# paipaoso/pytorch-operator-1

Hardware: AMD Instinct MI355X
Metric: samples/sec MNIST DDP (higher is better)
Workload: dtype fp32; 1 GPU; model=mnist-cnn (reference examples/mnist/mnist.py Net, 431,080 params), global_batch=64, per_rank_batch=64, optimizer=SGD lr=0.01 momentum=0.5, parallelism=dp1, impl=fused, sampler=none (every rank its own batch stream, reference-equivalent), backend=none

## Files before the change

### pytorch_operator_1_amd/csrc/kernels/mnist_kernels.hip

```cpp
#include <stdlib.h>

#include "mfma_f32.h"
#include "sgd_f32.h"
#include "xgmi_ar.h"

#ifndef PTO_STAMP
#define PTO_STAMP(k) ((void)0)
#define PTO_STAMP_SCOPE()
#endif

namespace {

constexpr int C1 = 20, C2 = 50, P1 = 12, F1OUT = 500, F1IN = 800, NCLS = 10;
constexpr int A1P = C1 * P1 * P1;

PTO_DEV void relu_pool4(const float v[4], float& out, uint8_t& code) {
  float m = v[0];
  int a = 0;
#pragma unroll
  for (int r = 1; r < 4; ++r)
    if (v[r] > m) { m = v[r]; a = r; }
  if (m > 0.f) { out = m; code = (uint8_t)a; }
  else { out = 0.f; code = 4; }
}
// ... 1232 lines not shown
          const bool ok = (unsigned)sy < 8u && (unsigned)sx < 8u;
          tv[kh * 5 + kw] = ts[(icl * 25 + kh * 5 + kw) * TLD + (ok ? sy * 8 + sx : 0)];
          tv[kh * 5 + kw] = ok ? tv[kh * 5 + kw] : 0.f;
        }
      float sacc = 0.f;
#pragma unroll
      for (int t = 0; t < 25; ++t) sacc += tv[t];
      if (da1p) da1p[b * A1P + (icg * 2 + icl) * 144 + pix] = sacc;
      dsum[o] = sacc;
    }
    {
      const int o = 256 + (tid >> 3), part = tid & 7, pix = o - 144;
      const int y = pix / 12, xx = pix - y * 12;
      float tv[4];
#pragma unroll
      for (int i = 0; i < 4; ++i) {
        const int tt = part + 8 * i;
        const int kh = tt / 5, kw = tt - kh * 5, sy = y - kh, sx = xx - kw;
        const bool ok = tt < 25 && (unsigned)sy < 8u && (unsigned)sx < 8u;
        tv[i] = ts[(25 + (tt < 25 ? tt : 0)) * TLD + (ok ? sy * 8 + sx : 0)];
        tv[i] = ok ? tv[i] : 0.f;
      }
      float sacc = tv[0];
      sacc += tv[1];
      sacc += tv[2];
      sacc += tv[3];
      sacc += lane_mirror8(sacc);
      sacc += lane_xor2(sacc);
      sacc += lane_xor1(sacc);
      if (part == 0) {
        if (da1p) da1p[b * A1P + (icg * 2 + 1) * 144 + pix] = sacc;
        dsum[o] = sacc;
      }
    }
  }
  if (!fuse1) return;
  __syncthreads();
  PTO_STAMP(4);
  float* part = ws;
  {
    const int icl = wv >> 1, p0 = (wv & 1) * 72;
    float acc[26];
#pragma unroll
    for (int k = 0; k < 26; ++k) acc[k] = 0.f;
#pragma unroll
    for (int it = 0; it < 2; ++it) {
      const int pl = lane + 64 * it;
      if (pl < 72) {
        const int pix = p0 + pl;
        const int cd = c1s[icl * 144 + pix];
        const float v = cd < 4 ? dsum[icl * 144 + pix] : 0.f;
        const int oh = 2 * (pix / 12) + ((cd >> 1) & 1), ow = 2 * (pix % 12) + (cd & 1);
        const float* xp = xs + oh * 28 + ow;
#pragma unroll
        for (int kh = 0; kh < 5; ++kh)
#pragma unroll
          for (int kw = 0; kw < 5; ++kw) acc[kh * 5 + kw] = fmaf(v, xp[kh * 28 + kw], acc[kh * 5 + kw]);
        acc[25] += v;
      }
    }
    wave_halving26(acc, lane, part + wv * 26);
  }
  __syncthreads();
  PTO_STAMP(5);
  if (tid < 52) {
    const int icl = tid / 26, k = tid - icl * 26, oc1 = icg * 2 + icl;
    const float v = part[(2 * icl) * 26 + k] + part[(2 * icl + 1) * 26 + k];
    if (det) {
      if (k < 25) gw1[oc1 * 25 + k] = v;
      else gb1[oc1] = v;
    } else {
      if (k < 25) atomicAdd(gw1 + oc1 * 25 + k, v);
      else atomicAdd(gb1 + oc1, v);
    }
  }
}

PTO_DEV float c2_bias_sum(int oc, const float* __restrict__ g2, const uint8_t* __restrict__ code2, int B) {
  const int lane = threadIdx.x & 63;
  float s = 0.f;
  for (int i0 = 0; i0 < B * 16; i0 += 64 * 8) {
    float gv[8];
    int cd[8];
#pragma unroll
    for (int q = 0; q < 8; ++q) {
      const int i = i0 + q * 64 + lane;
      const int idx = (i >> 4) * F1IN + oc * 16 + (i & 15);
      const bool ok = i < B * 16;
      gv[q] = ok ? g2[idx] : 0.f;
      cd[q] = ok ? (int)code2[idx] : 4;
    }
#pragma unroll
    for (int q = 0; q < 8; ++q) s += cd[q] < 4 ? gv[q] : 0.f;
  }
  return wave_sum(s);
}

__global__ __launch_bounds__(256) void k_conv2_bwd(const float* __restrict__ g2, const uint8_t* __restrict__ code2,
                                                   const float* __restrict__ a1p, const float* __restrict__ w2,
                                                   float* __restrict__ gw2, float* __restrict__ gb2,
                                                   float* __restrict__ da1p, int B, int nA, int nB, int nC,
                                                   const float* __restrict__ x, const long long* __restrict__ bidx,
                                                   const uint8_t* __restrict__ code1, float* __restrict__ gw1,
                                                   float* __restrict__ gb1) {
  extern __shared__ __attribute__((aligned(16))) float smem[];
  int bid = blockIdx.x;
  const int wv = threadIdx.x >> 6, lane = threadIdx.x & 63;
  if (bid < nA) {
    c2_wgrad_block<B2_CHUNK>(bid, smem, g2, code2, a1p, gw2, B);
    return;
  }
  bid -= nA;
  if (bid < nB) {
    c2_dgrad_block(bid, smem, g2, code2, w2, da1p, B, x, bidx, code1, gw1, gb1, false);
    return;
  }
  bid -= nB;
  if (bid < nC) {
    const int oc = bid * 4 + wv;
    if (oc >= C2) return;
    const float s = c2_bias_sum(oc, g2, code2, B);
    if (lane == 0) gb2[oc] = s;
  }
}

PTO_DEV void dw1_sgd_tile(int tile, const float* __restrict__ dh1, const float* __restrict__ a2p,
                          float* __restrict__ pw, float* __restrict__ mw, int B, const SgdArgs& a) {
  constexpr int MT = (F1OUT + 15) / 16, NT = (F1IN + 15) / 16;
  if (tile >= MT * NT) return;
  const int mt = tile % MT, nt = tile / MT, lane = threadIdx.x & 63;
  const int n = nt * 16 + (lane & 15);
  float pv[4], mv[4];
#pragma unroll
  for (int rr = 0; rr < 4; ++rr) {
    const int r = mt * 16 + (lane >> 4) * 4 + rr;
    const bool ok = r < F1OUT && n < F1IN;
    pv[rr] = ok ? pw[r * F1IN + n] : 0.f;
    mv[rr] = ok ? mw[r * F1IN + n] : 0.f;
  }
  const float lr = *a.lr;
  const f32x4 acc =
      wave_tile_16x16<LAY_KROW, LAY_KROW, 4>(dh1, F1OUT, a2p, F1IN, F1OUT, F1IN, B, mt * 16, nt * 16, 0, B);
#pragma unroll
  for (int rr = 0; rr < 4; ++rr) {
    const int r = mt * 16 + (lane >> 4) * 4 + rr;
    if (r < F1OUT && n < F1IN) {
      sgd_elem(pv[rr], acc[rr], mv[rr], lr, a.mom, a.wd, a.gscale, a.nesterov);
      pw[r * F1IN + n] = pv[rr];
      mw[r * F1IN + n] = mv[rr];
    }
  }
}

PTO_DEV void dw1_tile_pair(int pair, const float* __restrict__ dh1, const float* __restrict__ a2p,
                           float* __restrict__ pw, float* __restrict__ mw, float* __restrict__ gout, int B,
                           const SgdArgs& a) {
  constexpr int MT = (F1OUT + 15) / 16, NT = (F1IN + 15) / 16;
  static_assert(NT % 2 == 0 && F1IN % 16 == 0, "dW1 column tiles pair up with no column tail");
  if (pair >= MT * NT / 2) return;
  const int mt = pair % MT, nt0 = 2 * (pair / MT), lane = threadIdx.x & 63;
  const int r = lane & 15, g = lane >> 4;
  float pv[2][4], mv[2][4];
  if (!gout) {
#pragma unroll
    for (int t = 0; t < 2; ++t)
#pragma unroll
      for (int rr = 0; rr < 4; ++rr) {
        const int row = mt * 16 + g * 4 + rr, n = (nt0 + t) * 16 + r;
        const bool ok = row < F1OUT;
        pv[t][rr] = ok ? pw[row * F1IN + n] : 0.f;
        mv[t][rr] = ok ? mw[row * F1IN + n] : 0.f;
      }
  }
  f32x4 acc[2][2] = {{zero4(), zero4()}, {zero4(), zero4()}};
  constexpr int NG = 4;
  for (int k = 0; k < B; k += 16 * NG) {
    float av[NG][4], bv[2][NG][4];
#pragma unroll
    for (int q = 0; q < NG; ++q) {
      load4<LAY_KROW>(dh1, F1OUT, mt * 16 + r, F1OUT, k + 16 * q + 4 * g, B, av[q]);
#pragma unroll
      for (int t = 0; t < 2; ++t) load4<LAY_KROW>(a2p, F1IN, (nt0 + t) * 16 + r, F1IN, k + 16 * q + 4 * g, B, bv[t][q]);
    }
#pragma unroll
    for (int q = 0; q < NG; ++q)
#pragma unroll
      for (int j = 0; j < 4; ++j)
#pragma unroll
        for (int t = 0; t < 2; ++t) acc[t][j & 1] = mfma16x16x4(av[q][j], bv[t][q][j], acc[t][j & 1]);
  }
  const float lr = gout ? 0.f : *a.lr;
#pragma unroll
  for (int t = 0; t < 2; ++t) {
    const f32x4 s = acc[t][0] + acc[t][1];
#pragma unroll
    for (int rr = 0; rr < 4; ++rr) {
      const int row = mt * 16 + g * 4 + rr, n = (nt0 + t) * 16 + r;
      if (row >= F1OUT) continue;
      if (gout) {
        gout[row * F1IN + n] = s[rr];
      } else {
        sgd_elem(pv[t][rr], s[rr], mv[t][rr], lr, a.mom, a.wd, a.gscale, a.nesterov);
        pw[row * F1IN + n] = pv[t][rr];
        mw[row * F1IN + n] = mv[t][rr];
      }
    }
  }
}

constexpr int B1_CHUNK = 4;
PTO_DEV void conv1_bwd_block(int vb, const float* __restrict__ g1, const uint8_t* __restrict__ code1,
                             const float* __restrict__ x, float* __restrict__ gw1, float* __restrict__ gb1, int B,
                             const long long* __restrict__ bidx) {
  __shared__ __attribute__((aligned(16))) float xs[B1_CHUNK * 784];
  __shared__ float part[4][26];
  x = batch_ptr(x, bidx, B * 784);
  const int oc = vb % C1, chunk = vb / C1;
  const int b0 = chunk * B1_CHUNK, nb = min(B, b0 + B1_CHUNK) - b0;
  const int nitems = nb * 144;
  constexpr int PER = (B1_CHUNK * 144 + 255) / 256;
  constexpr int XPER = (B1_CHUNK * 196 + 255) / 256;
  float gv[PER];
  int cd[PER];
  float4 xv[XPER];
#pragma unroll
  for (int q = 0; q < XPER; ++q) {
    const int e = threadIdx.x + 256 * q;
    xv[q] = e < nb * 196 ? reinterpret_cast<const float4*>(x + b0 * 784)[e] : float4{0.f, 0.f, 0.f, 0.f};
  }
#pragma unroll
  for (int q = 0; q < PER; ++q) {
    const int it = threadIdx.x + 256 * q;
    const bool ok = it < nitems;
    const int idx = ok ? ((b0 + it / 144) * C1 + oc) * 144 + it % 144 : 0;
    gv[q] = ok ? g1[idx] : 0.f;
    cd[q] = ok ? (int)code1[idx] : 4;
  }
#pragma unroll
  for (int q = 0; q < XPER; ++q) {
    const int e = threadIdx.x + 256 * q;
    if (e < B1_CHUNK * 196) reinterpret_cast<float4*>(xs)[e] = xv[q];
  }
  __syncthreads();
  float acc[26];
#pragma unroll
  for (int k = 0; k < 26; ++k) acc[k] = 0.f;
#pragma unroll
  for (int q = 0; q < PER; ++q) {
    const int it = threadIdx.x + 256 * q;
    if (cd[q] >= 4) continue;
    const int smp = it / 144, pix = it - smp * 144;
    const int oh = 2 * (pix / 12) + (cd[q] >> 1), ow = 2 * (pix % 12) + (cd[q] & 1);
    const float* xp = xs + smp * 784 + oh * 28 + ow;
    const float gq = gv[q];
#pragma unroll
    for (int kh = 0; kh < 5; ++kh)
#pragma unroll
      for (int kw = 0; kw < 5; ++kw) acc[kh * 5 + kw] = fmaf(gq, xp[kh * 28 + kw], acc[kh * 5 + kw]);
    acc[25] += gq;
  }
  const int wv = threadIdx.x >> 6, lane = threadIdx.x & 63;
  wave_halving26(acc, lane, part[wv]);
  __syncthreads();
  if (threadIdx.x < 26) {
    const int q = threadIdx.x;
    const float s = part[0][q] + part[1][q] + part[2][q] + part[3][q];
    if (q < 25) atomicAdd(gw1 + oc * 25 + q, s);
    else atomicAdd(gb1 + oc, s);
  }
}

__global__ __launch_bounds__(256) void k_conv1_bwd(const float* __restrict__ g1, const uint8_t* __restrict__ code1,
                                                   const float* __restrict__ x, float* __restrict__ gw1,
                                                   float* __restrict__ gb1, int B,
                                                   const long long* __restrict__ bidx) {
  conv1_bwd_block(blockIdx.x, g1, code1, x, gw1, gb1, B, bidx);
}

#ifndef PTO_BWD_DTPW
#define PTO_BWD_DTPW 1
#endif
constexpr int BWD_DTPW = PTO_BWD_DTPW;
static int bwd_dpair() {
  static int v = -1;
  if (v < 0) {
    const char* e = getenv("PTO_BWD_DPAIR");
    v = (e && BWD_DTPW == 1) ? (atoi(e) != 0) : 0;
  }
  return v;
}
#ifndef PTO_BWD_ORDER
#define PTO_BWD_ORDER 0
#endif
__host__ __device__ constexpr int bwd_order(int i) {
  constexpr int o[6][5] = {{0, 1, 2, 3, 4}, {3, 2, 4, 0, 1}, {3, 2, 0, 1, 4}, {2, 3, 0, 1, 4},
                           {3, 4, 2, 0, 1}, {0, 1, 3, 2, 4}};
  return o[PTO_BWD_ORDER][i];
}
constexpr int bwd_n_dw1_blocks(bool pair) {
  return pair ? ((((F1OUT + 15) / 16) * ((F1IN + 15) / 16) / 2) + 3) / 4
              : ((((F1OUT + 15) / 16) * ((F1IN + 15) / 16) + 3) / 4 + BWD_DTPW - 1) / BWD_DTPW;
}

struct BwdAllArgs {
  const float* g2;
  const uint8_t* code2;
  const float* a1p;
  const float* w2f;
  const float* x;
  const uint8_t* code1;
  float* gw1;
  float* gb1;
  float* p2w; float* g2w; float* m2w;
  int* ctr;
  float* p2b; float* m2b;
  const float* dh1; const float* a2p; const float* h1; const float* dl;
  float* p1w; float* m1w;
  float* p1b; float* m1b;
  float* pfw; float* mfw;
  float* pfb; float* mfb;
  SgdArgs a;
  long long* bidx;
  long long nbatches;
  int* pending;
  int B, nA, nB, nC, nD, nF;
  int dpair;
  float* wpart;
  float* c1rep;
  int nrep, rep_stride, bias_off;
  int grads_only;
  float* g2b; float* g1w; float* g1b; float* gfw; float* gfb;
  float* hz;
  int nz;
};

struct EpiSgd {
  float* p; float* m; int ld; float lr; const SgdArgs* a;
  PTO_DEV void operator()(int r, int c, float g) const {
    const int i = r * ld + c;
    float pv = p[i], mv = m[i];
    sgd_elem(pv, g, mv, lr, a->mom, a->wd, a->gscale, a->nesterov);
    p[i] = pv;
    m[i] = mv;
  }
};

template <int CH, int NTW>
__global__ __launch_bounds__(256) void k_bwd_all(BwdAllArgs A) {
  extern __shared__ __attribute__((aligned(16))) float smem[];
  __shared__ int s_last;
  int bid = blockIdx.x;
  PTO_STAMP_SCOPE();
  const int wv = threadIdx.x >> 6, lane = threadIdx.x & 63;
  if (bid == 0 && threadIdx.x == 0) {
    if (A.bidx) *A.bidx = (*A.bidx + 1) % A.nbatches;
    if (A.pending) *A.pending = 1;
  }
  if (A.hz) {
    const int i = bid * 256 + (int)threadIdx.x;
    if (i < A.nz) A.hz[i] = 0.f;
  }
  int role = 4;
  {
    const int cnt[5] = {A.nC, A.nF, A.nA, A.nB, A.nD};
#pragma unroll
    for (int i = 0; i < 5; ++i) {
      const int r = bwd_order(i);
      if (bid < cnt[r]) {
        role = r;
        break;
      }
      bid -= cnt[r];
    }
  }
  if (role == 0) {
    const int oc = bid * 4 + wv;
    if (oc >= C2) return;
    const float g = c2_bias_sum(oc, A.g2, A.code2, A.B);
    if (lane == 0 && A.grads_only) A.g2b[oc] = g;
    else if (lane == 0) {
      float pv = A.p2b[oc], mv = A.m2b[oc];
      sgd_elem(pv, g, mv, *A.a.lr, A.a.mom, A.a.wd, A.a.gscale, A.a.nesterov);
      A.p2b[oc] = pv;
      A.m2b[oc] = mv;
    }
    return;
  }
  if (role == 1) {
    const float lr = *A.a.lr;
    constexpr int NWF = (((NCLS + 15) / 16) * ((F1OUT + 15) / 16) + 3) / 4;
    if (A.grads_only) {
      if (bid < NWF) {
        block_gemm_4tiles<LAY_KROW, LAY_KROW>(A.dl, NCLS, A.h1, F1OUT, NCLS, F1OUT, A.B, bid, EpiStore{A.gfw, F1OUT});
        return;
      }
      bid -= NWF;
      if (bid < 8) block_colsum64(A.dh1, F1OUT, A.B, F1OUT, bid * 64, smem, A.g1b);
      else block_colsum64(A.dl, NCLS, A.B, NCLS, 0, smem, A.gfb);
      return;
    }
    if (bid < NWF) {
      block_gemm_4tiles<LAY_KROW, LAY_KROW>(A.dl, NCLS, A.h1, F1OUT, NCLS, F1OUT, A.B, bid,
                                            EpiSgd{A.pfw, A.mfw, F1OUT, lr, &A.a});
      return;
    }
    bid -= NWF;
    if (bid < 8) block_colsum64_epi(A.dh1, F1OUT, A.B, F1OUT, bid * 64, smem, EpiSgd{A.p1b, A.m1b, 0, lr, &A.a});
    else block_colsum64_epi(A.dl, NCLS, A.B, NCLS, 0, smem, EpiSgd{A.pfb, A.mfb, 0, lr, &A.a});
    return;
  }
  if (role == 2) {
    const bool det = A.wpart != nullptr;
    c2_wgrad_block<CH, NTW>(bid, smem, A.g2, A.code2, A.a1p, A.g2w, A.B, A.wpart);
    if (A.grads_only && !det) return;
    asm volatile("s_waitcnt vmcnt(0)" ::: "memory");
    __syncthreads();
    PTO_STAMP(3);
    constexpr int NT = 32 / NTW, TC = 16 * NTW;
    const int nt = bid % NT, nchunk = A.nA / NT;
    if (threadIdx.x == 0) {
      if (det) __builtin_amdgcn_fence(__ATOMIC_RELEASE, "agent");
      const int old = __hip_atomic_fetch_add(A.ctr + nt, 1, __ATOMIC_RELAXED, __HIP_MEMORY_SCOPE_AGENT);
      s_last = old == nchunk - 1;
      if (s_last) {
        __hip_atomic_store(A.ctr + nt, 0, __ATOMIC_RELAXED, __HIP_MEMORY_SCOPE_AGENT);
        if (det) __builtin_amdgcn_fence(__ATOMIC_ACQUIRE, "agent");
      }
    }
    __syncthreads();
    PTO_STAMP(4);
    if (!s_last) return;
    constexpr int NQ = (C2 * TC + 255) / 256;
    int idx[NQ];
    float gv[NQ], pv[NQ], mv[NQ];
    if (det) {
#pragma unroll
      for (int q = 0; q < NQ; ++q) {
        const int e = threadIdx.x + 256 * q, row = e / TC, col = nt * TC + (e % TC);
        idx[q] = (e < C2 * TC && col < 500) ? row * 500 + col : -1;
        float g = 0.f;
        if (idx[q] >= 0)
          for (int c = 0; c < nchunk; ++c) g += A.wpart[c * (C2 * 500) + idx[q]];
        gv[q] = g;
      }
      if (A.grads_only) {
#pragma unroll
        for (int q = 0; q < NQ; ++q)
          if (idx[q] >= 0) A.g2w[idx[q]] = gv[q];
        return;
      }
    }
    const float lr = *A.a.lr;
#pragma unroll
    for (int q = 0; q < NQ; ++q) {
      const int e = threadIdx.x + 256 * q, row = e / TC, col = nt * TC + (e % TC);
      idx[q] = (e < C2 * TC && col < 500) ? row * 500 + col : -1;
      if (idx[q] >= 0) {
        if (!det) gv[q] = atomicExch(A.g2w + idx[q], 0.f);
        pv[q] = A.p2w[idx[q]];
        mv[q] = A.m2w[idx[q]];
      }
    }
#pragma unroll
    for (int q = 0; q < NQ; ++q)
      if (idx[q] >= 0) {
        sgd_elem(pv[q], gv[q], mv[q], lr, A.a.mom, A.a.wd, A.a.gscale, A.a.nesterov);
        A.p2w[idx[q]] = pv[q];
        A.m2w[idx[q]] = mv[q];
      }
    return;
  }
  if (role == 3) {
    const int r = (bid / B2_ICG) % A.nrep;
    float* gw1 = r == 0 ? A.gw1 : A.c1rep + (r - 1) * A.rep_stride;
    float* gb1 = r == 0 ? A.gb1 : A.c1rep + (r - 1) * A.rep_stride + A.bias_off;
    c2_dgrad_block(bid, smem, A.g2, A.code2, A.w2f, nullptr, A.B, A.x, nullptr, A.code1, gw1, gb1,
                   A.wpart != nullptr);
    return;
  }
  if (role == 4) {
    if (A.dpair) {
      dw1_tile_pair(bid * 4 + wv, A.dh1, A.a2p, A.p1w, A.m1w, A.grads_only ? A.g1w : nullptr, A.B, A.a);
      return;
    }
#pragma unroll
    for (int j = 0; j < BWD_DTPW; ++j) {
      const int vb = bid * BWD_DTPW + j;
      if (A.grads_only)
        block_gemm_4tiles<LAY_KROW, LAY_KROW, EpiStore, 4>(A.dh1, F1OUT, A.a2p, F1IN, F1OUT, F1IN, A.B, vb,
                                                          EpiStore{A.g1w, F1IN});
      else
        dw1_sgd_tile(vb * 4 + wv, A.dh1, A.a2p, A.p1w, A.m1w, A.B, A.a);
    }
    return;
  }
}

__global__ __launch_bounds__(256) void k_conv1_commit(Conv1Commit cm, int* __restrict__ pending) {
  const int pend = *cm.pending;
  const float lr = *cm.a.lr;
  if (!pend) return;
  for (int i = 4 * threadIdx.x; i < cm.n; i += 1024) commit4(cm, i, lr);
  __syncthreads();
  if (threadIdx.x == 0) *pending = 0;
}

__global__ __launch_bounds__(256) void k_ddp_sgd(float* __restrict__ p, float* __restrict__ g, float* __restrict__ m,
                                                 int n, int c1, int zero_from, float* __restrict__ rep, int nrep,
                                                 SgdArgs a, long long* __restrict__ bidx, long long nbatches) {
  if (bidx && blockIdx.x == 0 && threadIdx.x == 0) *bidx = (*bidx + 1) % nbatches;
  const int i = (blockIdx.x * 256 + threadIdx.x) * 4;
  if (i >= n) return;
  const float lr = *a.lr;
  if (i >= c1) {
    const Conv1Commit cm{p + c1, g + c1, m + c1, n - c1, nullptr, a, rep, nrep, n - c1};
    commit4(cm, i - c1, lr);
  } else {
    sgd_flat4(p, g, m, i, lr, a, i >= zero_from);
  }
}

__global__ __launch_bounds__(256) void k_conv1_bwd_data(const float* __restrict__ g1,
                                                        const uint8_t* __restrict__ code1,
                                                        const float* __restrict__ w, float* __restrict__ dx, int B) {
  const int idx = blockIdx.x * 256 + threadIdx.x;
  if (idx >= B * 784) return;
  const int b = idx / 784, pix = idx - b * 784, y = pix / 28, xx = pix - (pix / 28) * 28;
  float s = 0.f;
  for (int oc = 0; oc < C1; ++oc)
    for (int kh = 0; kh < 5; ++kh) {
      const int oh = y - kh;
      if (oh < 0 || oh >= 24) continue;
      for (int kw = 0; kw < 5; ++kw) {
        const int ow = xx - kw;
        if (ow < 0 || ow >= 24) continue;
        const int pi = ((b * C1 + oc) * 12 + (oh >> 1)) * 12 + (ow >> 1);
        if (code1[pi] == ((oh & 1) * 2 + (ow & 1))) s = fmaf(g1[pi], w[oc * 25 + kh * 5 + kw], s);
      }
    }
  dx[idx] = s;
}

__global__ __launch_bounds__(256) void k_eval_head(const float* __restrict__ logp, const int64_t* __restrict__ labels,
                                                   float* __restrict__ stats, int B) {
  const int row = blockIdx.x * 256 + threadIdx.x;
  float loss = 0.f, corr = 0.f;
  if (row < B) {
    const float* z = logp + row * NCLS;
    int am = 0;
    float mv = z[0];
    for (int c = 1; c < NCLS; ++c)
      if (z[c] > mv) { mv = z[c]; am = c; }
    const int y = (int)labels[row];
    loss = -z[y];
    corr = (am == y) ? 1.f : 0.f;
  }
  loss = wave_sum(loss);
  corr = wave_sum(corr);
  if ((threadIdx.x & 63) == 0) {
    atomicAdd(stats, loss);
    atomicAdd(stats + 1, corr);
  }
}

}

#define PTO_API extern "C" __attribute__((visibility("default")))
#define LAUNCH_CHECK() return (int)hipGetLastError()

PTO_API int pto_conv1_fwd(const float* x, const float* w, const float* b, float* out, uint8_t* code, int B,
                          const long long* bidx, hipStream_t s) {
  hipLaunchKernelGGL(k_conv1_fwd, dim3((B * 720 + 255) / 256), dim3(256), 0, s, x, w, b, out, code, B, bidx);
  LAUNCH_CHECK();
}

PTO_API int pto_conv2_fwd(const float* a1p, const float* w, const float* b, float* out, uint8_t* code, int B,
                          hipStream_t s) {
  hipLaunchKernelGGL(k_conv2_fwd, dim3(B * 4), dim3(256), 0, s, a1p, w, b, out, code, B);
  LAUNCH_CHECK();
}

static SgdArgs sgd_args(const float* lr, float mom, float wd, float gscale, int nesterov) {
  SgdArgs a;
  a.lr = lr;
  a.mom = mom;
  a.wd = wd;
  a.gscale = gscale;
  a.nesterov = nesterov;
  a.variant = 0;
  return a;
}

PTO_API int pto_conv12_fwd_lazy_x(const float* x, const float* w1, const float* b1, const float* w2,
                                  const float* b2, float* a1p, uint8_t* code1, float* a2p, uint8_t* code2, int B,
                                  const long long* bidx, const float* g1f, const float* m1f, int bias_off,
                                  const int* pending, const float* lr, float mom, float wd, float gscale, int nesterov,
                                  float* xout, float* w2out, const float* rep, int nrep, int rep_stride,
                                  hipStream_t s) {
  if (nrep < 1 || nrep > C1_MAXREP || (nrep > 1 && !rep) || (pending && (!g1f || !m1f || !lr))) return -1;
  LazyConv1 lz{g1f, m1f, pending, sgd_args(lr, mom, wd, gscale, nesterov), bias_off, xout, w2out, rep, nrep,
               rep_stride};
  hipLaunchKernelGGL(HIP_KERNEL_NAME(k_conv12_fwd2_t<1024, 0>), dim3(B * 4), dim3(1024), 0, s, x, w1, b1, w2, b2, a1p,
                     code1, a2p, code2, B, bidx, lz, ArRole{}, ArRole{});
  LAUNCH_CHECK();
}

extern "C" long long pto_ar_timeout_ticks();

PTO_API int pto_conv12_fwd_ar(const float* x, const float* w1, const float* b1, const float* w2, const float* b2,
                              float* a1p, uint8_t* code1, float* a2p, uint8_t* code2, int B, const long long* bidx,
                              float* xout, const void* peers, int rank, int world, void* epochs, void* err,
                              int protocol, float* p, float* m, const float* lr, float mom, float wd, float gscale,
                              int nesterov, long long fc_off, long long fc_n, int fc_chan, long long fc_zero_from,
                              long long cv_off, long long cv_n, int cv_chan, long long rep_base, int nrep,
                              int rep_stride, long long rep_from, int* ready, hipStream_t s) {
  using namespace pto_ar;
  if (fc_n <= AR_ONESHOT_MAX || fc_n % 4 || fc_off % 4 || fc_n > (1LL << 29) || cv_n > AR_ONESHOT_MAX || cv_n < 4 ||
      cv_n % 4 || cv_off % 4 || world < 1 || world > AR_MAX_RANKS || fc_chan < 0 || fc_chan >= AR_CHANNELS ||
      cv_chan < 0 || cv_chan >= AR_CHANNELS || fc_chan == cv_chan || rank < 0 || rank >= world || !p || !m || !lr ||
      !peers || !ready || protocol < 0 || protocol > 1 || B < 0 || ((((uintptr_t)p) | ((uintptr_t)m)) & 15))
    return -1;
  if (nrep < 1 || nrep > AR_MAX_REP || (nrep > 1 && (rep_stride % 4 || rep_from % 4 || rep_base % 4 ||
                                                      rep_base < cv_off + cv_n || rep_from < cv_off ||
                                                      rep_from + rep_stride > cv_off + cv_n)))
    return -1;
  LazyConv1 lz{nullptr, nullptr, nullptr, sgd_args(lr, mom, wd, gscale, nesterov), 0, xout, nullptr, nullptr, 1, 0};
  ArRole ar{}, cv{};
  for (ArRole* r : {&ar, &cv}) {
    r->peers = reinterpret_cast<const ArPeers*>(peers);
    r->rank = rank;
    r->world = world;
    r->epochs = reinterpret_cast<uint32_t*>(epochs);
    r->err = reinterpret_cast<int*>(err);
    r->timeout = pto_ar_timeout_ticks();
    r->f = ArSgd{};
    r->f.p = p;
    r->f.m = m;
    r->f.a = sgd_args(lr, mom, wd, gscale, nesterov);
    r->f.nbatches = 1;
    r->f.nrep = 1;
    r->ready = ready;
  }
  ar.off = fc_off;
  ar.n4 = fc_n / 4;
  ar.chan = fc_chan;
  ar.nblk = role_blocks(fc_n, world, 1024);
  ar.f.zero_from = fc_zero_from;
  cv.off = cv_off;
// ... 16 lines not shown
  LAUNCH_CHECK();
}

PTO_API int pto_linear_fwd(const float* x, const float* w, const float* b, float* y, int M, int N, int K, int relu,
                           hipStream_t s) {
  const int tiles = ((M + 15) / 16) * ((N + 15) / 16);
  const bool vec = (K % 4) == 0 && ((((uintptr_t)x) | ((uintptr_t)w)) & 15) == 0;
  if (vec)
    hipLaunchKernelGGL(k_linear_fwd_vec16, dim3(tiles), dim3(1024), 0, s, x, w, b, y, M, N, K, relu);
  else
    hipLaunchKernelGGL(k_linear_fwd, dim3(tiles), dim3(256), 0, s, x, w, b, y, M, N, K, relu);
  LAUNCH_CHECK();
}

PTO_API int pto_fc1_fwd_split(const float* x, const float* w, float* h, int M, hipStream_t s) {
  if (M < 1 || !x || !w || !h || ((((uintptr_t)x) | ((uintptr_t)w)) & 15)) return -1;
  static const int nw = [] {
    const char* e = getenv("PTO_FC1_NW");
    const int v = e ? atoi(e) : 16;
    return (v == 4 || v == 8) ? v : 16;
  }();
  const dim3 g(((M + 15) / 16) * 64);
  if (nw == 4)
    hipLaunchKernelGGL(HIP_KERNEL_NAME(k_fc1_fwd_split2<4>), g, dim3(256), 0, s, x, w, h, M);
  else if (nw == 16)
    hipLaunchKernelGGL(HIP_KERNEL_NAME(k_fc1_fwd_split2<16>), g, dim3(1024), 0, s, x, w, h, M);
  else
    hipLaunchKernelGGL(HIP_KERNEL_NAME(k_fc1_fwd_split2<8>), g, dim3(512), 0, s, x, w, h, M);
  LAUNCH_CHECK();
}

PTO_API int pto_linear_bwd(const float* dy, const float* x, const float* w, float* dx, float* dw, float* db, int M,
                           int N, int K, hipStream_t s) {
  if (dx) {
    const int tiles = ((M + 15) / 16) * ((K + 15) / 16);
    hipLaunchKernelGGL(k_linear_bwd_data, dim3(tiles), dim3(256), 0, s, dy, w, dx, M, N, K);
  }
  if (dw) {
    const int tiles = ((N + 15) / 16) * ((K + 15) / 16);
    hipLaunchKernelGGL(k_linear_bwd_weight, dim3((tiles + 3) / 4), dim3(256), 0, s, dy, x, dw, M, N, K);
  }
  if (db) hipLaunchKernelGGL(k_colsum, dim3((N + 63) / 64), dim3(256), 0, s, dy, db, M, N);
  LAUNCH_CHECK();
}

PTO_API int pto_relu_bwd(const float* g, const float* y, float* out, int n, hipStream_t s) {
  hipLaunchKernelGGL(k_relu_bwd, dim3((n + 255) / 256), dim3(256), 0, s, g, y, out, n);
  LAUNCH_CHECK();
}

PTO_API int pto_fc2_ce(const float* h1, const float* w, const float* b, const int64_t* labels, float* logp,
                       float* loss_rows, float* dlogits, float* dh1, int B, float inv_b, const long long* bidx,
                       hipStream_t s) {
  hipLaunchKernelGGL(k_fc2_ce, dim3((B + 3) / 4), dim3(256), 0, s, h1, w, b, labels, logp, loss_rows, dlogits, dh1,
                     B, inv_b, bidx);
  LAUNCH_CHECK();
}

PTO_API int pto_conv1_commit(float* p1, float* g1, float* m1, int n1, int* pending, const float* lr, float mom,
                             float wd, float gscale, int nesterov, float* rep, int nrep, int rep_stride,
                             hipStream_t s) {
  if (n1 % 4 || rep_stride % 4 || ((((uintptr_t)p1) | ((uintptr_t)g1) | ((uintptr_t)m1) | ((uintptr_t)rep)) & 15))
    return -1;
  Conv1Commit cm{p1, g1, m1, n1, pending, sgd_args(lr, mom, wd, gscale, nesterov), rep, nrep, rep_stride};
  hipLaunchKernelGGL(k_conv1_commit, dim3(1), dim3(256), 0, s, cm, pending);
  LAUNCH_CHECK();
}

PTO_API int pto_mnist_ddp_sgd(float* p, float* g, float* m, int n, int c1, int zero_from, float* rep, int nrep,
                              const float* lr, float mom, float wd, float gscale, int nesterov, long long* bidx,
                              long long nbatches, hipStream_t s) {
  if (n % 4 || c1 % 4 || zero_from % 4 || c1 < 0 || c1 >= n || !lr || nrep < 1 || nrep > C1_MAXREP ||
      (nrep > 1 && !rep) || (bidx && nbatches < 1))
    return -1;
  if ((((uintptr_t)p) | ((uintptr_t)g) | ((uintptr_t)m) | ((uintptr_t)rep)) & 15) return -1;
  hipLaunchKernelGGL(k_ddp_sgd, dim3((n / 4 + 255) / 256), dim3(256), 0, s, p, g, m, n, c1, zero_from, rep, nrep,
                     sgd_args(lr, mom, wd, gscale, nesterov), bidx, nbatches);
  LAUNCH_CHECK();
}

PTO_API int pto_conv2_bwd(const float* g2, const uint8_t* code2, const float* a1p, const float* w2, float* gw2,
                          float* gb2, float* da1p, int B, int parts, const float* x, const long long* bidx,
                          const uint8_t* code1, float* gw1, float* gb1, hipStream_t s) {
  if ((parts & 2) && (((uintptr_t)w2) & 7)) return -1;
  const int nA = (parts & 1) ? ((B + B2_CHUNK - 1) / B2_CHUNK) * 32 : 0;
  const int nB = (parts & 2) ? B * B2_ICG : 0;
  const int nC = (parts & 4) ? (C2 + 3) / 4 : 0;
  const size_t ldsA = (parts & 1) ? wgrad_lds_floats<B2_CHUNK, 1>() * sizeof(float) : 0;
  const size_t ldsB = (parts & 2) ? B2_LDS_FLOATS * sizeof(float) : 0;
  const size_t lds = ldsA > ldsB ? ldsA : ldsB;
  if (nA + nB + nC == 0) return 0;
  hipLaunchKernelGGL(k_conv2_bwd, dim3(nA + nB + nC), dim3(256), lds, s, g2, code2, a1p, w2, gw2, gb2, da1p, B, nA,
                     nB, nC, x, bidx, code1, (parts & 2) ? gw1 : nullptr, gb1);
  LAUNCH_CHECK();
}

PTO_API int pto_fc2_ce_dx(const float* h1, const float* w2, const float* b2, const int64_t* labels, const float* w1,
                          float* loss_rows, float* dlogits, float* dh1, float* da2p, int B, float inv_b,
                          const long long* bidx, float* p1, float* g1, float* m1, int n1, const int* pending,
                          const float* lr, float mom, float wd, float gscale, int nesterov, float* rep, int nrep,
                          int rep_stride, int* zero_word, const float* st_x, float* st_xnext, long long st_nb,
                          const float* b1, float* h1out, hipStream_t s) {
  if (b1 && (!h1out || ((((uintptr_t)b1) | ((uintptr_t)h1out)) & 15))) return -1;
  if (n1 % 4 || rep_stride % 4 || ((((uintptr_t)p1) | ((uintptr_t)g1) | ((uintptr_t)m1) | ((uintptr_t)rep)) & 15))
    return -1;
  if ((((uintptr_t)h1) | ((uintptr_t)w2)) & 15) return -1;
  if (nrep < 1 || nrep > C1_MAXREP || (nrep > 1 && !rep)) return -1;
  if (st_xnext && (!st_x || !bidx || st_nb < 1 || ((((uintptr_t)st_x) | ((uintptr_t)st_xnext)) & 15))) return -1;
  Conv1Commit cm{p1, g1, m1, n1, pending, sgd_args(lr, mom, wd, gscale, nesterov), rep, nrep, rep_stride, zero_word};
  const BatchStage st{st_x, st_xnext, st_nb, B * 784 / 4};
  const int nblk = ((B + 15) / 16) * ((F1IN + 15) / 16);
  hipLaunchKernelGGL(k_fc2_ce_dx_mf, dim3(nblk + 1 + (st_xnext ? STAGE_BLOCKS : 0)), dim3(FDX_WAVES * 64), 0, s, h1,
                     w2, b2, labels, w1, loss_rows, dlogits, dh1, da2p, B, inv_b, bidx, cm, st, b1, h1out);
  LAUNCH_CHECK();
}

PTO_API int pto_conv1_bwd(const float* g1, const uint8_t* code1, const float* x, float* gw1, float* gb1, int B,
                          const long long* bidx, hipStream_t s) {
  const int nblk = C1 * ((B + B1_CHUNK - 1) / B1_CHUNK);
  hipLaunchKernelGGL(k_conv1_bwd, dim3(nblk), dim3(256), 0, s, g1, code1, x, gw1, gb1, B, bidx);
  LAUNCH_CHECK();
}

PTO_API int pto_conv1_bwd_data(const float* g1, const uint8_t* code1, const float* w, float* dx, int B,
                               hipStream_t s) {
  hipLaunchKernelGGL(k_conv1_bwd_data, dim3((B * 784 + 255) / 256), dim3(256), 0, s, g1, code1, w, dx, B);
  LAUNCH_CHECK();
}

PTO_API int pto_eval_head(const float* logp, const int64_t* labels, float* stats, int B, hipStream_t s) {
  hipLaunchKernelGGL(k_eval_head, dim3((B + 255) / 256), dim3(256), 0, s, logp, labels, stats, B);
  LAUNCH_CHECK();
}

#ifndef PTO_BWD_WCHUNK
#define PTO_BWD_WCHUNK 5
#endif
constexpr int BWD_WCHUNK = PTO_BWD_WCHUNK;
constexpr int BWD_WNTW = 1;

PTO_API int pto_bwd_all(const float* g2, const uint8_t* code2, const float* a1p, const float* w2f, const float* x,
                        const uint8_t* code1, const float* dh1, const float* a2p, const float* h1, const float* dl,
                        float* p, float* g, float* m, long long off_fc2w, long long off_fc2b, long long off_fc1w,
                        long long off_fc1b, long long off_c2w, long long off_c2b, long long off_c1w,
                        long long off_c1b, int* ctr, long long* bidx, long long nbatches, int* pending, int B,
                        const float* lr, float mom, float wd, float gscale, int nesterov, float* c1rep, int nrep,
                        int rep_stride, int grads_only, float* wpart, float* hz, int nz, hipStream_t s) {
  if (!ctr) return -1;
  if (((uintptr_t)(grads_only ? p + off_c2w : w2f)) & 7) return -1;
  if (!grads_only && (!bidx || !pending || !w2f)) return -1;
  if (bidx && nbatches < 1) return -1;
  if (B < 1 || nrep < 1 || nrep > C1_MAXREP || (nrep > 1 && !c1rep)) return -1;
  if (wpart && nrep != B) return -1;
  BwdAllArgs A;
  A.g2 = g2; A.code2 = code2; A.a1p = a1p; A.w2f = w2f; A.x = x; A.code1 = code1;
  A.gw1 = g + off_c1w; A.gb1 = g + off_c1b;
  A.p2w = p + off_c2w; A.g2w = g + off_c2w; A.m2w = m + off_c2w; A.ctr = ctr;
  A.p2b = p + off_c2b; A.m2b = m + off_c2b;
  A.dh1 = dh1; A.a2p = a2p; A.h1 = h1; A.dl = dl;
  A.p1w = p + off_fc1w; A.m1w = m + off_fc1w;
  A.p1b = p + off_fc1b; A.m1b = m + off_fc1b;
  A.pfw = p + off_fc2w; A.mfw = m + off_fc2w;
  A.pfb = p + off_fc2b; A.mfb = m + off_fc2b;
  A.a = sgd_args(lr, mom, wd, gscale, nesterov);
  A.c1rep = c1rep;
  A.nrep = nrep;
  A.rep_stride = rep_stride;
  A.bias_off = (int)(off_c1b - off_c1w);
  A.grads_only = grads_only;
  A.g2b = g + off_c2b; A.g1w = g + off_fc1w; A.g1b = g + off_fc1b; A.gfw = g + off_fc2w; A.gfb = g + off_fc2b;
  if (grads_only) A.w2f = p + off_c2w;
  A.bidx = bidx; A.nbatches = nbatches; A.pending = pending; A.B = B;
  A.nA = ((B + BWD_WCHUNK - 1) / BWD_WCHUNK) * (32 / BWD_WNTW);
  A.nB = B * B2_ICG;
  A.nC = (C2 + 3) / 4;
  A.dpair = bwd_dpair();
  A.nD = bwd_n_dw1_blocks(A.dpair);
  A.nF = (((NCLS + 15) / 16) * ((F1OUT + 15) / 16) + 3) / 4 + 9;
  A.wpart = wpart;
  A.hz = hz;
  A.nz = hz ? nz : 0;
  if ((long long)A.nz > (long long)(A.nA + A.nB + A.nC + A.nD + A.nF) * 256) return -1;
  const size_t ldsA = wgrad_lds_floats<BWD_WCHUNK, BWD_WNTW>() * sizeof(float);
  const size_t ldsB = B2_LDS_FLOATS * sizeof(float);
  const size_t lds = ldsA > ldsB ? ldsA : ldsB;
  hipLaunchKernelGGL(HIP_KERNEL_NAME(k_bwd_all<BWD_WCHUNK, BWD_WNTW>), dim3(A.nA + A.nB + A.nC + A.nD + A.nF), dim3(256), lds, s, A);
  LAUNCH_CHECK();
}
```

### pytorch_operator_1_amd/ops/_lib.py

```python
from __future__ import annotations

import ctypes
import glob
import hashlib
import os
import shutil
import subprocess
import threading

PKG_DIR = os.path.dirname(os.path.dirname(os.path.abspath(__file__)))
CSRC = os.path.join(PKG_DIR, "csrc")
LIB_DIR = os.path.join(PKG_DIR, "_lib")
LIB_PATH = os.path.join(LIB_DIR, "libpto_hip.so")
ARCH = os.environ.get("PTO_OFFLOAD_ARCH", "gfx950")
HIPCC = os.environ.get("HIPCC", shutil.which("hipcc") or "/opt/rocm/bin/hipcc")

HIP_SOURCES = ("kernels/mnist_kernels.hip", "kernels/common_kernels.hip", "kernels/optim_kernels.hip",
               "kernels/llm_kernels.hip", "kernels/attention.hip", "kernels/bn_kernels.hip", "kernels/conv3x3.hip",
               "kernels/conv3x3_wgrad.hip", "kernels/gemm_bf16.hip", "comm/xgmi_allreduce.hip")

_lock = threading.Lock()
_RESTYPES = {"pto_ar_timeout_ticks": ctypes.c_longlong}
_lib = None


def _sources():
    return [os.path.join(CSRC, s) for s in HIP_SOURCES if os.path.exists(os.path.join(CSRC, s))]


def _digest() -> str:
    h = hashlib.sha256()
    h.update(ARCH.encode())
    for p in sorted(_sources() + glob.glob(os.path.join(CSRC, "kernels", "*.h")) +
                    glob.glob(os.path.join(CSRC, "comm", "*.h"))):
        with open(p, "rb") as f:
            h.update(f.read())
    return h.hexdigest()[:16]


def is_current() -> bool:
    stamp = LIB_PATH + ".stamp"
    if not (os.path.exists(LIB_PATH) and os.path.exists(stamp)):
        return False
    with open(stamp) as f:
        return f.read().strip() == _digest()


def build(force: bool = False, verbose: bool = False) -> str:
    os.makedirs(LIB_DIR, exist_ok=True)
    stamp = LIB_PATH + ".stamp"
    dig = _digest()
    if not force and os.path.exists(LIB_PATH) and os.path.exists(stamp):
        with open(stamp) as f:
            if f.read().strip() == dig:
                return LIB_PATH
    tmp = LIB_PATH + f".tmp{os.getpid()}"
    cmd = [HIPCC, f"--offload-arch={ARCH}", "-O3", "-std=c++17", "-fPIC", "-shared",
           "-I", os.path.join(CSRC, "kernels"), "-I", os.path.join(CSRC, "comm"), "-o", tmp] + _sources()
    if verbose:
        print(" ".join(cmd))
    subprocess.run(cmd, check=True)
    os.replace(tmp, LIB_PATH)
    with open(stamp, "w") as f:
        f.write(dig)
    return LIB_PATH


_P = ctypes.c_void_p
_I = ctypes.c_int
_F = ctypes.c_float
_L = ctypes.c_longlong

_SIGS = {
    "pto_conv1_fwd": [_P, _P, _P, _P, _P, _I, _P, _P],
    "pto_conv2_fwd": [_P, _P, _P, _P, _P, _I, _P],
    "pto_linear_fwd": [_P, _P, _P, _P, _I, _I, _I, _I, _P],
    "pto_linear_bwd": [_P, _P, _P, _P, _P, _P, _I, _I, _I, _P],
    "pto_relu_bwd": [_P, _P, _P, _I, _P],
    "pto_fc2_ce": [_P, _P, _P, _P, _P, _P, _P, _P, _I, _F, _P, _P],
    "pto_conv2_bwd": [_P, _P, _P, _P, _P, _P, _P, _I, _I, _P, _P, _P, _P, _P, _P],
    "pto_conv1_bwd": [_P, _P, _P, _P, _P, _I, _P, _P],
    "pto_conv1_bwd_data": [_P, _P, _P, _P, _I, _P],
    "pto_conv12_fwd_lazy_x": [_P] * 9 + [_I, _P, _P, _P, _I, _P, _P, _F, _F, _F, _I, _P, _P, _P, _I, _I, _P],
    "pto_conv12_fwd_ar": [_P] * 9 + [_I, _P, _P, _P, _I, _I, _P, _P, _I, _P, _P, _P, _F, _F, _F, _I,
                                     _L, _L, _I, _L, _L, _L, _I, _L, _I, _I, _L, _P, _P],
    "pto_synth_mnist": [_P, _P, _L, ctypes.c_ulonglong, _P],
    "pto_bwd_all": [_P] * 13 + [_L] * 8 + [_P, _P, _L, _P, _I, _P, _F, _F, _F, _I, _P, _I, _I, _I, _P, _P, _I,
                                          _P],
    "pto_conv1_commit": [_P, _P, _P, _I, _P, _P, _F, _F, _F, _I, _P, _I, _I, _P],
    "pto_mnist_ddp_sgd": [_P, _P, _P, _I, _I, _I, _P, _I, _P, _F, _F, _F, _I, _P, _L, _P],
    "pto_fc2_ce_dx": [_P] * 9 + [_I, _F, _P, _P, _P, _P, _I, _P, _P, _F, _F, _F, _I, _P, _I, _I, _P, _P, _P, _L,
                                  _P, _P, _P],
    "pto_fc1_fwd_split": [_P, _P, _P, _I, _P],
    "pto_eval_head": [_P, _P, _P, _I, _P],
    "pto_sgd_block_count": [_L],
    "pto_sgd_multi": [_P, _P, _I, _I, _P, _F, _F, _F, _F, _I, _I, _P, _L, _P],
    "pto_log_softmax_fwd": [_P, _P, _I, _I, _P],
    "pto_log_softmax_bwd": [_P, _P, _P, _I, _I, _P],
    "pto_cross_entropy_fwd": [_P, _P, _P, _P, _I, _I, _F, _P],
    "pto_scale": [_P, _P, _F, _L, _P],
    "pto_sum": [_P, _P, _L, _F, _P],
    "pto_adamw_block_count": [_L],
    "pto_adamw_multi": [_P, _P, _I, _I, _I, _P, _F, _F, _F, _F, _F, _I, _F, _I, _P],
    "pto_bf16_to_f32": [_P, _P, _L, _P],
    "pto_add_rmsnorm_fwd": [_P, _P, _P, _P, _P, _P, _L, _I, _F, _P],
    "pto_rmsnorm_bwd_groups": [_L],
    "pto_rmsnorm_bwd": [_P, _P, _P, _P, _P, _P, _P, _P, _L, _I, _P],
    "pto_swiglu_fwd": [_P, _P, _L, _I, _P],
    "pto_swiglu_bwd": [_P, _P, _P, _L, _I, _P],
    "pto_swiglu_bwd_t": [_P, _P, _P, _P, _L, _I, _P],
    "pto_rope": [_P, _P, _P, _P, _L, _I, _I, _I, _I, _L, _I, _P],
    "pto_ce_fwd": [_P, _P, _P, _P, _L, _I, _L, _P],
    "pto_ce_bwd": [_P, _P, _P, _P, _L, _I, _L, _P],
    "pto_transpose_bf16": [_P, _P, _L, _L, _L, _L, _P],
    "pto_noop": [_I, _P],
    "pto_graph_upload": [_P, _P],
    "pto_lane_ops_selftest": [_P, _P, _P, _P],
    "pto_probe_kernel": [_I, _I, _P, _I, _I, _P],
    "pto_gridbar_probe": [_I, _I, _P, _I, _I, _P],
    "pto_cu_id_probe": [_I, _P, _I, _P],
    "pto_stream_create_cu_mask": [ctypes.c_uint, _P, ctypes.POINTER(ctypes.c_void_p)],
    "pto_stream_get_cu_mask": [_P, ctypes.c_uint, _P],
    "pto_stream_destroy": [_P],
    "pto_bn_scratch_floats": [_L, _I],
    "pto_bn_fwd": [_P, _P, _P, _L, _I, _P, _P, _F, _F, _P, _P, _P, _P, _P, _I, _P, _P],
    "pto_bn_bwd": [_P, _P, _P, _P, _P, _L, _I, _P, _P, _P, _P, _P, _P, _I, _P],
    "pto_bn_fwd_part": [_P, _I, _P, _P, _P, _L, _I, _P, _P, _F, _F, _P, _P, _P, _P, _I, _P, _P],
    "pto_conv3x3_tile_m": [_I],
    "pto_conv3x3_set_variant": [_I, _I],
    "pto_conv3x3_fwd": [_P, _P, _P, _P, _I, _I, _I, _I, _I, _I, _P],
    "pto_conv1x1_fwd": [_P, _P, _P, _P, _I, _I, _I, _I, _I, _I, _P],
    "pto_conv1x1_set_variant": [_I],
    "pto_conv3x3_wcast": [_P, _P, _L, _P],
    "pto_conv3x3_wflip": [_P, _P, _P, _I, _I, _P],
    "pto_conv3x3_wgrad_splits": [_I, _I, _I, _I, _I, _I],
    "pto_conv3x3_wgrad": [_P, _P, _P, _P, _I, _I, _I, _I, _I, _I, _P],
    "pto_gemm_bf16": [_I, _P, _L, _P, _L, _P, _L, _I, _L, _L, _L, _P],
    "pto_gemm_bf16_supported": [_I, _L, _L, _L, _L, _L, _L],
    "pto_maxpool_fwd": [_P, _P, _P, _I, _I, _I, _I, _I, _I, _I, _I, _I, _P],
    "pto_stem_fwd": [_P, _P, _L, _L, _L, _L, _P, _P, _I, _P],
    "pto_maxpool_bwd": [_P, _P, _P, _I, _I, _I, _I, _I, _I, _I, _I, _I, _P],
    "pto_attn_fwd": [_P, _P, _P, _P, _P, _I, _I, _I, _I, _L, _L, _L, _L, _F, _P],
    "pto_attn_bwd": [_P, _P, _P, _P, _P, _P, _P, _P, _P, _P, _L, _I, _I, _I, _I, _L, _L, _L, _L, _F, _P],
    "pto_ar_ipc_handle_size": [],
    "pto_ar_flag_bytes": [_I],
    "pto_ar_max_ranks": [],
    "pto_ar_peers_bytes": [],
    "pto_ar_epoch_words": [],
    "pto_ar_set_timeout_ms": [_I],
    "pto_ar_set_protocol": [_I],
    "pto_ar_get_protocol": [],
    "pto_ar_alloc_flags": [ctypes.POINTER(ctypes.c_void_p)],
    "pto_ar_free": [_P],
    "pto_ar_get_ipc_handle": [_P, _P, ctypes.POINTER(ctypes.c_longlong)],
    "pto_ar_open_ipc_handle": [_P, ctypes.POINTER(ctypes.c_void_p)],
    "pto_ar_close_ipc_handle": [_P],
    "pto_ar_blocks": [_L, _I],
    "pto_ar_hash_offset_words": [],
    "pto_ar_hash_ring": [],
    "pto_ar_param_hash": [_P, _P, _L, _I, _I, _P, _P],
    "pto_ar_read_words": [_P, _P, _L],
    "pto_ar_read_words_async": [_P, _P, _L, _P],
    "pto_ar_allreduce": [_P, _L, _L, _I, _I, _I, _P, _P, _P],
    "pto_ar_timeout_ticks": [],
    "pto_ar_allreduce_bf16": [_P, _L, _L, _I, _I, _I, _P, _P, _P],
    "pto_ar_role_sgd": [_P, _L, _L, _I, _I, _I, _P, _P, _I, _P, _P, _P, _F, _F, _F, _I, _L, _P],
    "pto_ar_oneshot_role_sgd": [_P, _L, _L, _I, _I, _I, _P, _P, _I, _P, _P, _P, _F, _F, _F, _I, _L, _I, _I, _L, _P,
                                _P],
    "pto_ar_oneshot_role_blocks": [_L, _I],
    "pto_ar_allreduce_sgd": [_P, _L, _L, _I, _I, _I, _P, _P, _P, _P, _P, _F, _F, _F, _I, _L, _P, _L, _P, _I, _I, _L,
                             _P],
}


def _current_library() -> str:
    try:
        return build(force=os.environ.get("PTO_REBUILD") == "1")
    except (OSError, subprocess.CalledProcessError):
        if not is_current():
            raise
        return LIB_PATH


def lib():
    global _lib
    if _lib is not None:
        return _lib
    with _lock:
        if _lib is not None:
            return _lib
        path = os.environ.get("PTO_HIP_LIB") or _current_library()
        L = ctypes.CDLL(path)
        for name, args in _SIGS.items():
            fn = getattr(L, name, None)
            if fn is None:
                continue
            fn.argtypes = args
            fn.restype = _RESTYPES.get(name, ctypes.c_int)
        _lib = L
        return _lib


def loaded_path() -> str | None:
    return getattr(_lib, "_name", None) if _lib is not None else None


def check(rc: int, what: str) -> None:
    if rc != 0:
        raise RuntimeError(f"{what} failed with hipError {rc}")


def stream_ptr(device=None) -> int:
    import torch

    return torch.cuda.current_stream(device).cuda_stream


def ptr(t) -> int | None:
    return None if t is None else t.data_ptr()
```

Measured before the change: 1.870 million samples/s.

## Transpose dW1 tile mapping for float4 SGD updates and XCD-aware block ids

Adds a transposed dW1 tile routine so each lane owns four contiguous columns, turning the fused SGD read-modify-write of fc1 weights and momentum into float4 loads and buffer stores with a cache-policy bit. Block ids for the heavier roles (dW, conv2 dgrad, dW1) are remapped so consecutive logical blocks land on the same XCD, aiming for better L2 locality on MI355X's chiplet layout. It also adds a standalone dW1 kernel and a block-map query for testing, plus a 16-byte alignment check on the fc1 buffers that makes the call fail otherwise.

```diff
diff --git a/pytorch_operator_1_amd/csrc/kernels/mnist_kernels.hip b/pytorch_operator_1_amd/csrc/kernels/mnist_kernels.hip
--- a/pytorch_operator_1_amd/csrc/kernels/mnist_kernels.hip
+++ b/pytorch_operator_1_amd/csrc/kernels/mnist_kernels.hip
@@ -1408,6 +1408,43 @@
   }
 }
 
+PTO_DEV void st4_wt(float* base, int i, float4 v) {
+  constexpr int AUX_SC1 = 16;
+  __builtin_amdgcn_raw_buffer_store_b128(__builtin_bit_cast(pto_ar::v4u, v),
+                                         pto_ar::mkbuf(base, (long long)F1OUT * F1IN * 4).r, i * 4, 0, AUX_SC1);
+}
+
+PTO_DEV void dw1_tile_t(int tile, const float* __restrict__ dh1, const float* __restrict__ a2p,
+                        float* __restrict__ pw, float* __restrict__ mw, float* __restrict__ gout, int B,
+                        const SgdArgs& a) {
+  constexpr int MT = (F1OUT + 15) / 16, NT = (F1IN + 15) / 16;
+  static_assert(F1IN % 16 == 0, "a lane's four columns never cross the row end");
+  if (tile >= MT * NT) return;
+  const int mt = tile % MT, nt = tile / MT, lane = threadIdx.x & 63;
+  const int row = mt * 16 + (lane & 15);
+  const bool ok = row < F1OUT;
+  const int i = (ok ? row : 0) * F1IN + nt * 16 + (lane >> 4) * 4;
+  float4 pv = {0.f, 0.f, 0.f, 0.f}, mv = pv;
+  if (!gout) {
+    pv = *reinterpret_cast<const float4*>(pw + i);
+    mv = *reinterpret_cast<const float4*>(mw + i);
+  }
+  const float lr = gout ? 0.f : *a.lr;
+  const f32x4 acc =
+      wave_tile_16x16<LAY_KROW, LAY_KROW, 4>(a2p, F1IN, dh1, F1OUT, F1IN, F1OUT, B, nt * 16, mt * 16, 0, B);
+  if (!ok) return;
+  if (gout) {
+    *reinterpret_cast<float4*>(gout + i) = float4{acc[0], acc[1], acc[2], acc[3]};
+    return;
+  }
+  sgd_elem(pv.x, acc[0], mv.x, lr, a.mom, a.wd, a.gscale, a.nesterov);
+  sgd_elem(pv.y, acc[1], mv.y, lr, a.mom, a.wd, a.gscale, a.nesterov);
+  sgd_elem(pv.z, acc[2], mv.z, lr, a.mom, a.wd, a.gscale, a.nesterov);
+  sgd_elem(pv.w, acc[3], mv.w, lr, a.mom, a.wd, a.gscale, a.nesterov);
+  st4_wt(pw, i, pv);
+  st4_wt(mw, i, mv);
+}
+
 PTO_DEV void dw1_tile_pair(int pair, const float* __restrict__ dh1, const float* __restrict__ a2p,
                            float* __restrict__ pw, float* __restrict__ mw, float* __restrict__ gout, int B,
                            const SgdArgs& a) {
@@ -1552,6 +1589,29 @@
   constexpr int o[6][5] = {{0, 1, 2, 3, 4}, {3, 2, 4, 0, 1}, {3, 2, 0, 1, 4}, {2, 3, 0, 1, 4},
                            {3, 4, 2, 0, 1}, {0, 1, 3, 2, 4}};
   return o[PTO_BWD_ORDER][i];
+}
+__host__ __device__ inline int bwd_xcd_id(int bid, int o, int T) {
+  const int x = (o + bid) & 7;
+  int base = 0;
+  for (int s = 0; s < x; ++s) {
+    const int d = (s - o) & 7;
+    base += d < T ? ((T - 1 - d) >> 3) + 1 : 0;
+  }
+  return base + (bid >> 3);
+}
+__host__ __device__ inline int bwd_role_id(int gid, const int cnt[5], int* id) {
+  int o = 0;
+#pragma unroll
+  for (int i = 0; i < 5; ++i) {
+    const int r = bwd_order(i);
+    if (gid - o < cnt[r]) {
+      *id = r >= 2 ? bwd_xcd_id(gid - o, o, cnt[r]) : gid - o;
+      return r;
+    }
+    o += cnt[r];
+  }
+  *id = gid - o;
+  return -1;
 }
 constexpr int bwd_n_dw1_blocks(bool pair) {
   return pair ? ((((F1OUT + 15) / 16) * ((F1IN + 15) / 16) / 2) + 3) / 4
@@ -1616,19 +1676,8 @@
     const int i = bid * 256 + (int)threadIdx.x;
     if (i < A.nz) A.hz[i] = 0.f;
   }
-  int role = 4;
-  {
-    const int cnt[5] = {A.nC, A.nF, A.nA, A.nB, A.nD};
-#pragma unroll
-    for (int i = 0; i < 5; ++i) {
-      const int r = bwd_order(i);
-      if (bid < cnt[r]) {
-        role = r;
-        break;
-      }
-      bid -= cnt[r];
-    }
-  }
+  const int cnt[5] = {A.nC, A.nF, A.nA, A.nB, A.nD};
+  const int role = bwd_role_id(blockIdx.x, cnt, &bid);
   if (role == 0) {
     const int oc = bid * 4 + wv;
     if (oc >= C2) return;
@@ -1735,21 +1784,27 @@
     return;
   }
   if (role == 4) {
+    float* const gout = A.grads_only ? A.g1w : nullptr;
     if (A.dpair) {
-      dw1_tile_pair(bid * 4 + wv, A.dh1, A.a2p, A.p1w, A.m1w, A.grads_only ? A.g1w : nullptr, A.B, A.a);
+      dw1_tile_pair(bid * 4 + wv, A.dh1, A.a2p, A.p1w, A.m1w, gout, A.B, A.a);
       return;
     }
 #pragma unroll
-    for (int j = 0; j < BWD_DTPW; ++j) {
-      const int vb = bid * BWD_DTPW + j;
-      if (A.grads_only)
-        block_gemm_4tiles<LAY_KROW, LAY_KROW, EpiStore, 4>(A.dh1, F1OUT, A.a2p, F1IN, F1OUT, F1IN, A.B, vb,
-                                                          EpiStore{A.g1w, F1IN});
-      else
-        dw1_sgd_tile(vb * 4 + wv, A.dh1, A.a2p, A.p1w, A.m1w, A.B, A.a);
-    }
+    for (int j = 0; j < BWD_DTPW; ++j)
+      dw1_tile_t((bid * BWD_DTPW + j) * 4 + wv, A.dh1, A.a2p, A.p1w, A.m1w, gout, A.B, A.a);
     return;
   }
+}
+
+__global__ __launch_bounds__(256) void k_dw1_tiles(const float* __restrict__ dh1, const float* __restrict__ a2p,
+                                                   float* __restrict__ pw, float* __restrict__ mw,
+                                                   float* __restrict__ gout, int B, SgdArgs a, int form) {
+  const int bid = blockIdx.x, wv = threadIdx.x >> 6;
+  if (form == 2) dw1_tile_pair(bid * 4 + wv, dh1, a2p, pw, mw, gout, B, a);
+  else if (form == 1) dw1_tile_t(bid * 4 + wv, dh1, a2p, pw, mw, gout, B, a);
+  else if (gout)
+    block_gemm_4tiles<LAY_KROW, LAY_KROW, EpiStore, 4>(dh1, F1OUT, a2p, F1IN, F1OUT, F1IN, B, bid, EpiStore{gout, F1IN});
+  else dw1_sgd_tile(bid * 4 + wv, dh1, a2p, pw, mw, B, a);
 }
 
 __global__ __launch_bounds__(256) void k_conv1_commit(Conv1Commit cm, int* __restrict__ pending) {
@@ -2072,6 +2127,8 @@
   if (bidx && nbatches < 1) return -1;
   if (B < 1 || nrep < 1 || nrep > C1_MAXREP || (nrep > 1 && !c1rep)) return -1;
   if (wpart && nrep != B) return -1;
+  if ((((uintptr_t)(p + off_fc1w)) | ((uintptr_t)(g + off_fc1w)) | ((uintptr_t)(m + off_fc1w))) & 15)
+    return -1;
   BwdAllArgs A;
   A.g2 = g2; A.code2 = code2; A.a1p = a1p; A.w2f = w2f; A.x = x; A.code1 = code1;
   A.gw1 = g + off_c1w; A.gb1 = g + off_c1b;
@@ -2107,3 +2164,25 @@
   hipLaunchKernelGGL(HIP_KERNEL_NAME(k_bwd_all<BWD_WCHUNK, BWD_WNTW>), dim3(A.nA + A.nB + A.nC + A.nD + A.nF), dim3(256), lds, s, A);
   LAUNCH_CHECK();
 }
+
+PTO_API int pto_bwd_block_map(int B, int dpair, int* role, int* id, int cap) {
+  if (B < 1) return -1;
+  const int cnt[5] = {(C2 + 3) / 4, (((NCLS + 15) / 16) * ((F1OUT + 15) / 16) + 3) / 4 + 9,
+                      ((B + BWD_WCHUNK - 1) / BWD_WCHUNK) * (32 / BWD_WNTW), B * B2_ICG,
+                      bwd_n_dw1_blocks(dpair != 0 && BWD_DTPW == 1)};
+  const int n = cnt[0] + cnt[1] + cnt[2] + cnt[3] + cnt[4];
+  if (n > cap) return -1;
+  for (int i = 0; i < n; ++i) role[i] = bwd_role_id(i, cnt, id + i);
+  return n;
+}
+
+PTO_API int pto_dw1_tiles(const float* dh1, const float* a2p, float* pw, float* mw, float* gout, int B,
+                          const float* lr, float mom, float wd, float gscale, int nesterov, int form,
+                          hipStream_t s) {
+  if (B < 1 || form < 0 || form > 2 || (!gout && (!pw || !mw || !lr))) return -1;
+  if ((((uintptr_t)pw) | ((uintptr_t)mw) | ((uintptr_t)gout)) & 15) return -1;
+  const int nblk = form == 2 ? bwd_n_dw1_blocks(true) : (((F1OUT + 15) / 16) * ((F1IN + 15) / 16) + 3) / 4;
+  hipLaunchKernelGGL(k_dw1_tiles, dim3(nblk), dim3(256), 0, s, dh1, a2p, pw, mw, gout, B,
+                     sgd_args(lr, mom, wd, gscale, nesterov), form);
+  LAUNCH_CHECK();
+}
diff --git a/pytorch_operator_1_amd/ops/_lib.py b/pytorch_operator_1_amd/ops/_lib.py
--- a/pytorch_operator_1_amd/ops/_lib.py
+++ b/pytorch_operator_1_amd/ops/_lib.py
@@ -87,6 +87,8 @@
     "pto_synth_mnist": [_P, _P, _L, ctypes.c_ulonglong, _P],
     "pto_bwd_all": [_P] * 13 + [_L] * 8 + [_P, _P, _L, _P, _I, _P, _F, _F, _F, _I, _P, _I, _I, _I, _P, _P, _I,
                                           _P],
+    "pto_bwd_block_map": [_I, _I, _P, _P, _I],
+    "pto_dw1_tiles": [_P, _P, _P, _P, _P, _I, _P, _F, _F, _F, _I, _I, _P],
     "pto_conv1_commit": [_P, _P, _P, _I, _P, _P, _F, _F, _F, _I, _P, _I, _I, _P],
     "pto_mnist_ddp_sgd": [_P, _P, _P, _I, _I, _I, _P, _I, _P, _F, _F, _F, _I, _P, _L, _P],
     "pto_fc2_ce_dx": [_P] * 9 + [_I, _F, _P, _P, _P, _P, _I, _P, _P, _F, _F, _F, _I, _P, _I, _I, _P, _P, _P, _L,
```

After: 1.924 million samples/s (median of 6 runs). 1.03x the previous value.
